# MiniMax-AI/VTP

Measured on AMD Instinct MI355X. Metric: images/sec/node VTP-B f16d64 256x256 train step, higher is better.
Workload: dtype bf16

## Files before the change

### vtp_amd/csrc/attention_resident.hip

```cpp
#include "common.h"
#include <algorithm>
#include <cstdio>
#include <cstdlib>
#include "vtp_hip.h"

namespace vtp {

constexpr float LOG2E_R = 1.4426950408889634f;
constexpr float LN2_R = 0.6931471805599453f;
constexpr int RES_MAXN = 320;
constexpr int RES_SPLIT_COLS = 4;

struct AttnResArgs {
  const bf16 *q, *k, *v, *o, *d_o;
  bf16 *out, *dq, *dk, *dv;
  float* lse;
  float* delta;
  const bf16 *rope_sin, *rope_cos;
  int rope_prefix;
  int B, N, heads, npad;
  long sb, sn, sbo, sno;
  float scale;
  int stagger;
  long long* timing;
// ... 142 lines not shown
  stage_resident(p.k + (long)b * p.sb + h * 64, p.sn, p.N, p.npad, Ks, wave, nwaves, lane);
  stage_resident(p.v + (long)b * p.sb + h * 64, p.sn, p.N, p.npad, Vs, wave, nwaves, lane);
  wait_vmcnt_upto(((p.npad >> 3) - wave + nwaves - 1) / nwaves);
  __builtin_amdgcn_s_barrier();
  asm volatile("" ::: "memory");
  const float sc2 = p.scale * LOG2E_R;
  const int nkb = p.npad >> 5, last = nkb - 1;
  float mx = -INFINITY;
  for (int kb = 0; kb < (active ? nkb : 0); ++kb) {
    f32x16 s;
    zero16r(s);
#pragma unroll
    for (int ks = 0; ks < 4; ++ks) s = __builtin_amdgcn_mfma_f32_32x32x16_bf16(frag_row(Ks, kb * 32, ks, lane), qf[ks], s, 0, 0, 0);
    if (kb == last) {
#pragma unroll
      for (int r = 0; r < 16; ++r)
        if (kb * 32 + (r & 3) + 8 * (r >> 2) + 4 * hi >= p.N) s[r] = -INFINITY;
    }
#pragma unroll
    for (int r = 0; r < 16; ++r) mx = fmaxf(mx, s[r]);
  }
  mx = fmaxf(mx, __shfl_xor(mx, 32, 64));
  const float m2 = mx * sc2;
  wait_all_dma();
  __syncthreads();
  if (!active) return;
  f32x16 oacc[2];
  zero16r(oacc[0]);
  zero16r(oacc[1]);
  float l = 0.f;
  for (int kb = 0; kb < nkb; ++kb) {
    f32x16 s;
    zero16r(s);
#pragma unroll
    for (int ks = 0; ks < 4; ++ks) s = __builtin_amdgcn_mfma_f32_32x32x16_bf16(frag_row(Ks, kb * 32, ks, lane), qf[ks], s, 0, 0, 0);
#pragma unroll
    for (int r = 0; r < 16; ++r) s[r] = fast_exp2(s[r] * sc2 - m2);
    if (kb == last) {
#pragma unroll
      for (int r = 0; r < 16; ++r)
        if (kb * 32 + (r & 3) + 8 * (r >> 2) + 4 * hi >= p.N) s[r] = 0.f;
    }
#pragma unroll
    for (int r = 0; r < 16; ++r) l += s[r];
    const bf16x8 pf0 = pack8r(s, 0), pf1 = pack8r(s, 8);
#pragma unroll
    for (int db = 0; db < 2; ++db) {
      oacc[db] = __builtin_amdgcn_mfma_f32_32x32x16_bf16(frag_tr(Vs, db, kb * 32, 0, lane), pf0, oacc[db], 0, 0, 0);
      oacc[db] = __builtin_amdgcn_mfma_f32_32x32x16_bf16(frag_tr(Vs, db, kb * 32, 1, lane), pf1, oacc[db], 0, 0, 0);
    }
  }
  l += __shfl_xor(l, 32, 64);
  if (qi >= p.N) return;
  const float inv = 1.f / l;
  bf16* orow = p.out + (long)b * p.sbo + (long)qi * p.sno + h * 64;
#pragma unroll
  for (int db = 0; db < 2; ++db)
#pragma unroll
    for (int g = 0; g < 4; ++g) {
      f32x4 v;
#pragma unroll
      for (int e = 0; e < 4; ++e) v[e] = oacc[db][4 * g + e] * inv;
      *(bf16x4*)(orow + db * 32 + 8 * g + 4 * hi) = __builtin_convertvector(v, bf16x4);
    }
  if (hi == 0 && p.lse) p.lse[((long)b * p.heads + h) * p.N + qi] = (m2 + log2f(l)) * LN2_R;
}

__device__ __forceinline__ float both_halves_sum(float x) {
  const auto r = __builtin_amdgcn_permlane32_swap(__float_as_uint(x), __float_as_uint(x), false, false);
  return __uint_as_float(r[0]) + __uint_as_float(r[1]);
}

__device__ __forceinline__ float max3f(float a, float b, float c) {
  float r;
  asm("v_max3_f32 %0, %1, %2, %3" : "=v"(r) : "v"(a), "v"(b), "v"(c));
  return r;
}
__device__ __forceinline__ float max2f(float a, float b) {
  float r;
  asm("v_max_f32 %0, %1, %2" : "=v"(r) : "v"(a), "v"(b));
  return r;
}

constexpr float LAZY_LOG2 = 6.f;

template <int T>
__device__ __forceinline__ void attn_key_loop(const char* Ks, const char* Vs, const bf16x8 (&qf)[T][4], int N, int nkb, int kb0, int step,
                                              float sc2, int lane, f32x16 (&oacc)[T][2], float (&m)[T], float (&l)[T],
                                              int stream_ops = 0) {
  const int hi = lane >> 5, last = nkb - 1;
  const f32x16 zero = {0.f, 0.f, 0.f, 0.f, 0.f, 0.f, 0.f, 0.f, 0.f, 0.f, 0.f, 0.f, 0.f, 0.f, 0.f, 0.f};
  const f32x2 sc2v = {sc2, sc2};
#pragma unroll
  for (int t = 0; t < T; ++t) {
    oacc[t][0] = zero;
    oacc[t][1] = zero;
    m[t] = -INFINITY;
    l[t] = 0.f;
  }
  for (int kb = kb0; kb < nkb; kb += step) {
    if (stream_ops > 0 && (kb == 2 || kb == 5)) {
      wait_vmcnt_upto(__builtin_amdgcn_readfirstlane(kb == 2 ? stream_ops * max(nkb - 5, 0) : 0));
      __builtin_amdgcn_s_barrier();
      asm volatile("" ::: "memory");
    }
    f32x16 s[T];
    {
      bf16x8 kf[4];
#pragma unroll
      for (int ks = 0; ks < 4; ++ks) kf[ks] = frag_row(Ks, kb * 32, ks, lane);
#pragma unroll
      for (int t = 0; t < T; ++t) {
        s[t] = __builtin_amdgcn_mfma_f32_32x32x16_bf16(kf[0], qf[t][0], zero, 0, 0, 0);
#pragma unroll
        for (int ks = 1; ks < 4; ++ks) s[t] = __builtin_amdgcn_mfma_f32_32x32x16_bf16(kf[ks], qf[t][ks], s[t], 0, 0, 0);
      }
    }
    bf16x8 vf[2][2];
#pragma unroll
    for (int db = 0; db < 2; ++db)
#pragma unroll
      for (int ks = 0; ks < 2; ++ks) vf[db][ks] = frag_tr(Vs, db, kb * 32, ks, lane);
    if (kb == last && (N & 31)) {
#pragma unroll
      for (int t = 0; t < T; ++t)
#pragma unroll
        for (int r = 0; r < 16; ++r)
          if (kb * 32 + (r & 3) + 8 * (r >> 2) + 4 * hi >= N) s[t][r] = -INFINITY;
    }
    float mn[T];
    bool moved = false;
#pragma unroll
    for (int t = 0; t < T; ++t) {
      float bm = max3f(s[t][0], s[t][1], s[t][2]);
#pragma unroll
      for (int r = 3; r < 15; r += 2) bm = max3f(bm, s[t][r], s[t][r + 1]);
      bm = max2f(bm, s[t][15]);
      const auto sw = __builtin_amdgcn_permlane32_swap(__float_as_uint(bm), __float_as_uint(bm), false, false);
      bm = max2f(__uint_as_float(sw[0]), __uint_as_float(sw[1]));
      const float cand = bm * sc2;
      mn[t] = cand > m[t] + LAZY_LOG2 ? cand : m[t];
      moved |= mn[t] > m[t];
    }
    if (__any(moved)) {
#pragma unroll
      for (int t = 0; t < T; ++t) {
        const float alpha = fast_exp2(m[t] - mn[t]);
        l[t] *= alpha;
        oacc[t][0] *= alpha;
        oacc[t][1] *= alpha;
        m[t] = mn[t];
      }
    }
    bf16x8 pf[T][2];
#pragma unroll
    for (int t = 0; t < T; ++t) {
      const f32x2 mv = {-m[t], -m[t]};
      f32x2 acc = {0.f, 0.f};
#pragma unroll
      for (int i = 0; i < 8; ++i) {
        f32x2 v = {s[t][2 * i], s[t][2 * i + 1]};
        v = __builtin_elementwise_fma(v, sc2v, mv);
        v[0] = fast_exp2(v[0]);
        v[1] = fast_exp2(v[1]);
        acc += v;
        s[t][2 * i] = v[0];
        s[t][2 * i + 1] = v[1];
      }
      l[t] += acc[0] + acc[1];
      pf[t][0] = pack8r(s[t], 0);
      pf[t][1] = pack8r(s[t], 8);
    }
#pragma unroll
    for (int db = 0; db < 2; ++db)
#pragma unroll
      for (int ks = 0; ks < 2; ++ks) {
#pragma unroll
        for (int t = 0; t < T; ++t) oacc[t][db] = __builtin_amdgcn_mfma_f32_32x32x16_bf16(vf[db][ks], pf[t][ks], oacc[t][db], 0, 0, 0);
      }
  }
}

__device__ __forceinline__ void store_o_row(bf16* orow, const f32x16 (&o)[2], float inv, int hi, bool valid) {
#pragma unroll
  for (int db = 0; db < 2; ++db)
#pragma unroll
    for (int j = 0; j < 2; ++j) {
      uint32_t x[2], y[2];
#pragma unroll
      for (int w = 0; w < 2; ++w) {
        const f32x2 vx = {o[db][8 * j + 2 * w] * inv, o[db][8 * j + 2 * w + 1] * inv};
        const f32x2 vy = {o[db][8 * j + 4 + 2 * w] * inv, o[db][8 * j + 4 + 2 * w + 1] * inv};
        const bf16x2 bx = __builtin_convertvector(vx, bf16x2), by = __builtin_convertvector(vy, bf16x2);
        x[w] = __builtin_bit_cast(uint32_t, bx);
        y[w] = __builtin_bit_cast(uint32_t, by);
      }
      uint32_t out[4];
#pragma unroll
      for (int w = 0; w < 2; ++w) {
        const auto r = __builtin_amdgcn_permlane32_swap(x[w], y[w], false, false);
        out[w] = r[0];
        out[2 + w] = r[1];
      }
      if (valid) {
        typedef __attribute__((ext_vector_type(4))) uint32_t u32x4;
        *(u32x4*)(orow + db * 32 + 16 * j + 8 * hi) = u32x4{out[0], out[1], out[2], out[3]};
      }
    }
}

__device__ __forceinline__ void stage_piece_asm(const bf16* base, long sn, int N, int piece, unsigned img_off, int lane) {
  const int row = piece * 8 + (lane >> 3);
  const int c = (lane & 7) ^ swz_key(row);
  const unsigned voff = (unsigned)(min(row, N - 1) * (int)sn + c * 8) * 2u;
  const unsigned dst = __builtin_amdgcn_readfirstlane(img_off + piece * 1024);
  unsigned keep;
  asm volatile("s_mov_b32 %0, m0\n\ts_mov_b32 m0, %3\n\ts_nop 0\n\tglobal_load_lds_dwordx4 %1, %2\n\ts_mov_b32 m0, %0"
               : "=&s"(keep)
               : "v"(voff), "s"(base), "s"(dst)
               : "memory");
}
__device__ __forceinline__ void stage_block_asm(const bf16* kbase, const bf16* vbase, long sn, int N, int kb, unsigned img, int wave,
                                                int nwaves, int lane) {
  for (int j = wave; j < 4; j += nwaves) {
    stage_piece_asm(kbase, sn, N, kb * 4 + j, 0, lane);
    stage_piece_asm(vbase, sn, N, kb * 4 + j, img, lane);
  }
}

#define ATTN_TSTAMP(i)                                                                            \
  do {                                                                                            \
    if (p.delta && blockIdx.x == 3 && blockIdx.y == 5 && lane == 0)                               \
      ((long long*)p.delta)[wave * 8 + (i)] = __builtin_readcyclecounter();                       \
  } while (0)

__global__ __launch_bounds__(256, 2) void attn_fwd_res2_kernel(const AttnResArgs p) {
  extern __shared__ __attribute__((aligned(16))) char smem[];
  char* Ks = smem;
  char* Vs = smem + p.npad * 128;
  float* part = (float*)(smem + 2 * p.npad * 128);
  const int lane = threadIdx.x & 63, wave = threadIdx.x >> 6, nwaves = blockDim.x >> 6, hi = lane >> 5;
  const int h = blockIdx.x, b = blockIdx.y;
  const bf16* qb = p.q + (long)b * p.sb + h * 64;
  const int ntiles = p.npad >> 5, nkb = ntiles, q0 = wave * 64;
  ATTN_TSTAMP(0);
  const bool split_last = (ntiles & 1) && ntiles > 1;
  const int qL = (ntiles - 1) * 32;
  bf16x8 qf[2][4], qfl[1][4];
#pragma unroll
  for (int t = 0; t < 2; ++t) {
    const bf16* qr = qb + (long)min(q0 + 32 * t + (lane & 31), p.N - 1) * p.sn + hi * 8;
#pragma unroll
    for (int ks = 0; ks < 4; ++ks) qf[t][ks] = *(const bf16x8*)(qr + ks * 16);
  }
  if (split_last) {
    const bf16* qr = qb + (long)min(qL + (lane & 31), p.N - 1) * p.sn + hi * 8;
#pragma unroll
    for (int ks = 0; ks < 4; ++ks) qfl[0][ks] = *(const bf16x8*)(qr + ks * 16);
  }
  const bf16* kbase = p.k + (long)b * p.sb + h * 64;
  const bf16* vbase = p.v + (long)b * p.sb + h * 64;
  const unsigned img = p.npad * 128;
  stage_block_asm(kbase, vbase, p.sn, p.N, 0, img, wave, nwaves, lane);
  if (nkb > 1) stage_block_asm(kbase, vbase, p.sn, p.N, 1, img, wave, nwaves, lane);
  __builtin_amdgcn_s_waitcnt(0x0F70);
  ATTN_TSTAMP(1);
  __builtin_amdgcn_s_barrier();
  asm volatile("" ::: "memory");
  ATTN_TSTAMP(2);
  for (int kb = 2; kb < nkb; ++kb) stage_block_asm(kbase, vbase, p.sn, p.N, kb, img, wave, nwaves, lane);
  const int stream_ops = 2 * ((4 - wave + nwaves - 1) / nwaves);
  const float sc2 = p.scale * LOG2E_R;
  const long srow0 = ((long)b * p.heads + h) * p.N;
  {
    f32x16 oacc[2][2];
    float m[2], l[2];
    const bool two = q0 + 32 < p.npad && !(split_last && q0 + 32 >= qL);
    if (two) attn_key_loop<2>(Ks, Vs, qf, p.N, nkb, 0, 1, sc2, lane, oacc, m, l, stream_ops);
    else {
      f32x16 (&o1)[1][2] = *(f32x16(*)[1][2])&oacc;
      attn_key_loop<1>(Ks, Vs, *(const bf16x8(*)[1][4])&qf, p.N, nkb, 0, 1, sc2, lane, o1, *(float(*)[1])&m, *(float(*)[1])&l,
                       stream_ops);
    }
    ATTN_TSTAMP(3);
#pragma unroll
    for (int t = 0; t < 2; ++t) {
      if (t == 1 && !two) break;
      const int qi = q0 + 32 * t + (lane & 31);
      const float lt = both_halves_sum(l[t]);
      const bool valid = qi < p.N;
      store_o_row(p.out + (long)b * p.sbo + (long)min(qi, p.N - 1) * p.sno + h * 64, oacc[t], 1.f / lt, hi, valid);
      if (valid && hi == 0 && p.lse) p.lse[srow0 + qi] = (m[t] + log2f(lt)) * LN2_R;
    }
  }
  ATTN_TSTAMP(4);
  if (!split_last) return;
  const int cols = p.N - qL;
  {
    f32x16 oacc[1][2];
    float m[1], l[1];
    attn_key_loop<1>(Ks, Vs, qfl, p.N, nkb, wave, nwaves, sc2, lane, oacc, m, l);
    const float lt = both_halves_sum(l[0]);
    if ((lane & 31) < cols) {
      float* dst = part + ((wave * cols + (lane & 31)) * 2 + hi) * 34;
      dst[0] = m[0];
      dst[1] = lt;
#pragma unroll
      for (int r = 0; r < 16; ++r) {
        dst[2 + r] = oacc[0][0][r];
        dst[18 + r] = oacc[0][1][r];
      }
    }
  }
  ATTN_TSTAMP(5);
  __syncthreads();
  ATTN_TSTAMP(6);
  if (wave != 0) return;
  {
    const int c = min(lane & 31, cols - 1);
    float M = -INFINITY;
    for (int w = 0; w < nwaves; ++w) M = fmaxf(M, part[((w * cols + c) * 2 + hi) * 34]);
    f32x16 o[2];
    zero16r(o[0]);
    zero16r(o[1]);
    float L = 0.f;
    for (int w = 0; w < nwaves; ++w) {
      const float* src = part + ((w * cols + c) * 2 + hi) * 34;
      const float sc = fast_exp2(src[0] - M);
      L += src[1] * sc;
#pragma unroll
      for (int r = 0; r < 16; ++r) {
        o[0][r] += src[2 + r] * sc;
        o[1][r] += src[18 + r] * sc;
      }
    }
    const int qi = qL + (lane & 31);
    const bool valid = (lane & 31) < cols;
    store_o_row(p.out + (long)b * p.sbo + (long)min(qi, p.N - 1) * p.sno + h * 64, o, 1.f / L, hi, valid);
    if (valid && hi == 0 && p.lse) p.lse[srow0 + qi] = (M + log2f(L)) * LN2_R;
  }
}

__global__ __launch_bounds__(640) void attn_bwd_dq_res_kernel(const AttnResArgs p) {
  extern __shared__ __attribute__((aligned(16))) char smem[];
  char* Ks = smem;
  char* Vs = smem + p.npad * 128;
  const int lane = threadIdx.x & 63, wave = threadIdx.x >> 6, nwaves = blockDim.x >> 6, hi = lane >> 5;
  const int h = blockIdx.x, b = blockIdx.y;
  BWD_STAMP(0);
  if (__builtin_expect(p.stagger > 0, 0)) {
    const int wg = (blockIdx.z * gridDim.y + blockIdx.y) * gridDim.x + blockIdx.x;
    if (wg < 256 && ((wg >> 3) & 1)) {
      const unsigned long long t0 = wall_clock64();
      while (wall_clock64() - t0 < (unsigned long long)p.stagger) __builtin_amdgcn_s_sleep(16);
    }
  }
  stage_resident(p.k + (long)b * p.sb + h * 64, p.sn, p.N, p.npad, Ks, wave, nwaves, lane);
  stage_resident(p.v + (long)b * p.sb + h * 64, p.sn, p.N, p.npad, Vs, wave, nwaves, lane);
  const int q0 = (blockIdx.z * nwaves + wave) * 32, qi = q0 + (lane & 31), qc = min(qi, p.N - 1);
  bf16x8 qf[4], dof[4];
  {
    const bf16* qr = p.q + (long)b * p.sb + h * 64 + (long)qc * p.sn + hi * 8;
    const bf16* gr = p.d_o + (long)b * p.sbo + h * 64 + (long)qc * p.sno + hi * 8;
#pragma unroll
    for (int ks = 0; ks < 4; ++ks) {
      qf[ks] = *(const bf16x8*)(qr + ks * 16);
      dof[ks] = *(const bf16x8*)(gr + ks * 16);
    }
  }
  const long srow = ((long)b * p.heads + h) * p.N + qc;
  const float lse2 = p.lse[srow] * LOG2E_R;
  float dlt = 0.f;
  {
    const bf16* orow = p.o + (long)b * p.sbo + h * 64 + (long)qc * p.sno + hi * 8;
#pragma unroll
    for (int ks = 0; ks < 4; ++ks) {
      const bf16x8 ov = *(const bf16x8*)(orow + ks * 16);
#pragma unroll
      for (int e = 0; e < 8; ++e) dlt += bf2f(ov[e]) * bf2f(dof[ks][e]);
    }
    dlt += __shfl_xor(dlt, 32, 64);
    if (hi == 0 && qi < p.N) p.delta[srow] = dlt;
  }
  wait_all_dma();
  __syncthreads();
  BWD_STAMP(1);
  if (q0 >= p.npad) return;
  const float sc2 = p.scale * LOG2E_R;
  const f32x2 sc2v = {sc2, sc2}, nlse = {-lse2, -lse2}, scv = {p.scale, p.scale}, ndlt = {-dlt * p.scale, -dlt * p.scale};
  const int nkb = p.npad >> 5, last = nkb - 1;
  f32x16 dq[2];
  zero16r(dq[0]);
  zero16r(dq[1]);
  for (int kb = 0; kb < nkb; ++kb) {
    f32x16 s, dp;
    zero16r(s);
    zero16r(dp);
#pragma unroll
    for (int ks = 0; ks < 4; ++ks) {
      s = __builtin_amdgcn_mfma_f32_32x32x16_bf16(frag_row(Ks, kb * 32, ks, lane), qf[ks], s, 0, 0, 0);
      dp = __builtin_amdgcn_mfma_f32_32x32x16_bf16(frag_row(Vs, kb * 32, ks, lane), dof[ks], dp, 0, 0, 0);
    }
#pragma unroll
    for (int i = 0; i < 8; ++i) {
      f32x2 e = {s[2 * i], s[2 * i + 1]}, g = {dp[2 * i], dp[2 * i + 1]};
      e = __builtin_elementwise_fma(e, sc2v, nlse);
      g = __builtin_elementwise_fma(g, scv, ndlt);
      e[0] = fast_exp2(e[0]);
      e[1] = fast_exp2(e[1]);
      e *= g;
      s[2 * i] = e[0];
      s[2 * i + 1] = e[1];
    }
    if (kb == last && (p.N & 31)) {
#pragma unroll
      for (int r = 0; r < 16; ++r)
        if (kb * 32 + (r & 3) + 8 * (r >> 2) + 4 * hi >= p.N) s[r] = 0.f;
    }
    const bf16x8 d0 = pack8r(s, 0), d1 = pack8r(s, 8);
#pragma unroll
    for (int db = 0; db < 2; ++db) {
      dq[db] = __builtin_amdgcn_mfma_f32_32x32x16_bf16(frag_tr(Ks, db, kb * 32, 0, lane), d0, dq[db], 0, 0, 0);
      dq[db] = __builtin_amdgcn_mfma_f32_32x32x16_bf16(frag_tr(Ks, db, kb * 32, 1, lane), d1, dq[db], 0, 0, 0);
    }
// ... 191 lines not shown
#pragma unroll
  for (int ks = 0; ks < 4; ++ks)
#pragma unroll
    for (int e = 0; e < 8; ++e) dlt += bf2f(of[ks][e]) * bf2f(dof[ks][e]);
  return dlt + __shfl_xor(dlt, 32, 64);
}

#define PB_STAMP(i)                                                                                                   \
  do {                                                                                                                \
    if (__builtin_expect(p.timing != nullptr, 0) && lane == 0) p.timing[((size_t)hid * 16 + wave) * 4 + (i)] = wall_clock64(); \
  } while (0)

__device__ __forceinline__ void dkv_step(const bf16x8 (&kf)[4], const bf16x8 (&vf)[4], f32x16 (&dk)[2], f32x16 (&dv)[2],
                                         const int (&rpart)[4], const int (&tpart)[2][2], int qoff, int img, const float* lse_s,
                                         const float* dlt_s, f32x2 sc2v, f32x2 scv, int q0, int N, bool mask, int hi) {
  f32x16 s, dp;
  zero16r(s);
  zero16r(dp);
#pragma unroll
  for (int ks = 0; ks < 4; ++ks) {
    s = __builtin_amdgcn_mfma_f32_32x32x16_bf16(frag_row_at(lds_addr(rpart[ks], qoff)), kf[ks], s, 0, 0, 0);
    dp = __builtin_amdgcn_mfma_f32_32x32x16_bf16(frag_row_at(lds_addr(rpart[ks], qoff + img)), vf[ks], dp, 0, 0, 0);
  }
  f32x16 pr;
#pragma unroll
  for (int g = 0; g < 4; ++g) {
    const f32x4 l4 = *(const f32x4*)(lse_s + q0 + 8 * g + 4 * hi);
    const f32x4 d4 = *(const f32x4*)(dlt_s + q0 + 8 * g + 4 * hi);
#pragma unroll
    for (int e2 = 0; e2 < 2; ++e2) {
      const int r = 4 * g + 2 * e2;
      f32x2 e = {s[r], s[r + 1]}, gq = {dp[r], dp[r + 1]};
      e = __builtin_elementwise_fma(e, sc2v, f32x2{l4[2 * e2], l4[2 * e2 + 1]});
      gq = __builtin_elementwise_fma(gq, scv, f32x2{d4[2 * e2], d4[2 * e2 + 1]});
      e[0] = fast_exp2(e[0]);
      e[1] = fast_exp2(e[1]);
      if (mask) {
        if (q0 + 8 * g + 4 * hi + 2 * e2 >= N) e[0] = 0.f;
        if (q0 + 8 * g + 4 * hi + 2 * e2 + 1 >= N) e[1] = 0.f;
      }
      pr[r] = e[0];
      pr[r + 1] = e[1];
      e *= gq;
      s[r] = e[0];
      s[r + 1] = e[1];
    }
  }
  const bf16x8 p0 = pack8r(pr, 0), p1 = pack8r(pr, 8), d0 = pack8r(s, 0), d1 = pack8r(s, 8);
#pragma unroll
  for (int db = 0; db < 2; ++db) {
    const int tq0 = lds_addr(tpart[db][0], qoff), tq1 = lds_addr(tpart[db][1], qoff);
    const int tg0 = lds_addr(tpart[db][0], qoff + img), tg1 = lds_addr(tpart[db][1], qoff + img);
    dv[db] = __builtin_amdgcn_mfma_f32_32x32x16_bf16(frag_tr_at(tg0, tg1, 0), p0, dv[db], 0, 0, 0);
    dv[db] = __builtin_amdgcn_mfma_f32_32x32x16_bf16(frag_tr_at(tg0, tg1, 1), p1, dv[db], 0, 0, 0);
    dk[db] = __builtin_amdgcn_mfma_f32_32x32x16_bf16(frag_tr_at(tq0, tq1, 0), d0, dk[db], 0, 0, 0);
    dk[db] = __builtin_amdgcn_mfma_f32_32x32x16_bf16(frag_tr_at(tq0, tq1, 1), d1, dk[db], 0, 0, 0);
  }
}

__device__ __forceinline__ void put_slot(float* slot, const f32x16 (&acc)[2], int hi) {
#pragma unroll
  for (int db = 0; db < 2; ++db)
#pragma unroll
    for (int g = 0; g < 4; ++g) {
      f32x4 v;
#pragma unroll
      for (int e = 0; e < 4; ++e) v[e] = acc[db][4 * g + e];
      *(f32x4*)(slot + 32 * db + 8 * g + 4 * hi) = v;
    }
}
__device__ __forceinline__ void store_acc_rows(bf16* row, const f32x16 (&acc)[2], int hi, const bf16* sin_t, const bf16* cos_t, long t) {
#pragma unroll
  for (int g = 0; g < 4; ++g) {
    f32x4 lo, hv;
#pragma unroll
    for (int e = 0; e < 4; ++e) {
      lo[e] = acc[0][4 * g + e];
      hv[e] = acc[1][4 * g + e];
    }
    store_grad_pair(row, 8 * g + 4 * hi, lo, hv, sin_t, cos_t, t);
  }
}

template <int W>
__global__ __launch_bounds__(64 * W) void attn_bwd_fused_kernel(const AttnResArgs p) {
  extern __shared__ __attribute__((aligned(16))) char smem[];
  const int lane = threadIdx.x & 63, wave = threadIdx.x >> 6, hi = lane >> 5;
  const int img = p.npad * 128, nb = p.npad >> 5, last = nb - 1;
  const bool odd = nb > W;
  const int nx = odd ? p.N - 32 * W : 0;
  const int QO = 0, KO = img, VO = 2 * img, GO = 3 * img;
  float* lse_s = (float*)(smem + 4 * img);
  float* dlt_s = lse_s + p.npad;
  float* xq = dlt_s + p.npad;
  float* xk = xq + (W + 1) * PB_XROWS * 64;
  float* xv = xk + (W + 1) * PB_XROWS * 64;
  const int hid = blockIdx.x, b = hid / p.heads, h = hid - b * p.heads;
  PB_STAMP(0);
  stage_image_asm(p.q + (long)b * p.sb + h * 64, p.sn, p.N, p.npad, QO, wave, W, lane);
  stage_image_asm(p.d_o + (long)b * p.sbo + h * 64, p.sno, p.N, p.npad, GO, wave, W, lane);
  stage_image_asm(p.k + (long)b * p.sb + h * 64, p.sn, p.N, p.npad, KO, wave, W, lane);
  stage_image_asm(p.v + (long)b * p.sb + h * 64, p.sn, p.N, p.npad, VO, wave, W, lane);
  const float sc2 = p.scale * LOG2E_R;
  const f32x2 sc2v = {sc2, sc2}, scv = {p.scale, p.scale};
  int rpart[4], tpart[2][2];
#pragma unroll
  for (int ks = 0; ks < 4; ++ks) rpart[ks] = row_part(lane) ^ (ks << 5);
#pragma unroll
  for (int db = 0; db < 2; ++db)
#pragma unroll
    for (int hf = 0; hf < 2; ++hf) tpart[db][hf] = tr_part(lane, hf) ^ (db << 6);
  const long srow0 = ((long)b * p.heads + h) * p.N;
  const int ri = wave * 32 + (lane & 31);
  const int rx = 32 * W + (lane & 31);
  bf16x8 of[4], of2[4];
  float lse_raw, lse_raw2 = 0.f;
  {
    const int qc = min(ri, p.N - 1);
    const bf16* orow = p.o + (long)b * p.sbo + h * 64 + (long)qc * p.sno + hi * 8;
#pragma unroll
    for (int ks = 0; ks < 4; ++ks) of[ks] = *(const bf16x8*)(orow + ks * 16);
    lse_raw = p.lse[srow0 + qc];
    if (odd) {
      const int qc2 = min(rx, p.N - 1);
      const bf16* orow2 = p.o + (long)b * p.sbo + h * 64 + (long)qc2 * p.sno + hi * 8;
#pragma unroll
      for (int ks = 0; ks < 4; ++ks) of2[ks] = *(const bf16x8*)(orow2 + ks * 16);
      lse_raw2 = p.lse[srow0 + qc2];
    }
  }
  wait_all_dma();
  __syncthreads();
  PB_STAMP(1);
  {
    bf16x8 qf[4], dof[4];
    const int own = __builtin_amdgcn_readfirstlane(wave * 4096);
#pragma unroll
    for (int ks = 0; ks < 4; ++ks) {
      qf[ks] = frag_row_at(lds_addr(rpart[ks], QO + own));
      dof[ks] = frag_row_at(lds_addr(rpart[ks], GO + own));
    }
    const float dlt = row_delta(of, dof);
    if (hi == 0) {
      lse_s[ri] = -lse_raw * LOG2E_R;
      dlt_s[ri] = -dlt * p.scale;
      if (ri < p.N) p.delta[srow0 + ri] = dlt;
    }
    {
      const float lse2 = lse_raw * LOG2E_R;
      const f32x2 nlse = {-lse2, -lse2}, ndlt = {-dlt * p.scale, -dlt * p.scale};
      f32x16 dq[2];
      zero16r(dq[0]);
      zero16r(dq[1]);
      for (int kb = 0; kb < nb; ++kb)
        dq_step(qf, dof, dq, rpart, tpart, __builtin_amdgcn_readfirstlane(KO + kb * 4096), img, sc2v, nlse, scv, ndlt, kb * 32, p.N,
                kb == last && (p.N & 31), hi);
      if (ri < p.N) {
        const bool rot = p.rope_sin && ri >= p.rope_prefix;
        store_acc_rows(p.dq + (long)b * p.sb + (long)ri * p.sn + h * 64, dq, hi, rot ? p.rope_sin : nullptr, p.rope_cos,
                       (long)(ri - p.rope_prefix) * 64);
      }
    }
    if (odd) {
      const int ox = __builtin_amdgcn_readfirstlane(W * 4096);
#pragma unroll
      for (int ks = 0; ks < 4; ++ks) {
        qf[ks] = frag_row_at(lds_addr(rpart[ks], QO + ox));
        dof[ks] = frag_row_at(lds_addr(rpart[ks], GO + ox));
      }
      const float dlt2 = row_delta(of2, dof);
      if (wave == 0 && hi == 0) {
        lse_s[rx] = -lse_raw2 * LOG2E_R;
        dlt_s[rx] = -dlt2 * p.scale;
        if (rx < p.N) p.delta[srow0 + rx] = dlt2;
      }
      const float lse2 = lse_raw2 * LOG2E_R;
      const f32x2 nlse = {-lse2, -lse2}, ndlt = {-dlt2 * p.scale, -dlt2 * p.scale};
      for (int kb = wave; kb < nb; kb += W) {
        f32x16 dqx[2];
        zero16r(dqx[0]);
        zero16r(dqx[1]);
        dq_step(qf, dof, dqx, rpart, tpart, __builtin_amdgcn_readfirstlane(KO + kb * 4096), img, sc2v, nlse, scv, ndlt, kb * 32, p.N,
                kb == last && (p.N & 31), hi);
        if ((lane & 31) < nx) put_slot(xq + (kb * PB_XROWS + (lane & 31)) * 64, dqx, hi);
      }
    }
  }
  __syncthreads();
  PB_STAMP(2);
  if (odd && (int)threadIdx.x < nx * 8) {
    const int row = threadIdx.x >> 3, d0 = 4 * (threadIdx.x & 7), qrow = 32 * W + row;
    f32x4 lo = {0.f, 0.f, 0.f, 0.f}, hv = {0.f, 0.f, 0.f, 0.f};
    for (int kb = 0; kb < nb; ++kb) {
      lo += *(const f32x4*)(xq + (kb * PB_XROWS + row) * 64 + d0);
      hv += *(const f32x4*)(xq + (kb * PB_XROWS + row) * 64 + 32 + d0);
    }
    const bool rot = p.rope_sin && qrow >= p.rope_prefix;
    store_grad_pair(p.dq + (long)b * p.sb + (long)qrow * p.sn + h * 64, d0, lo, hv, rot ? p.rope_sin : nullptr, p.rope_cos,
                    (long)(qrow - p.rope_prefix) * 64);
  }
  {
    bf16x8 kf[4], vf[4];
    const int own = __builtin_amdgcn_readfirstlane(wave * 4096);
#pragma unroll
    for (int ks = 0; ks < 4; ++ks) {
      kf[ks] = frag_row_at(lds_addr(rpart[ks], KO + own));
      vf[ks] = frag_row_at(lds_addr(rpart[ks], VO + own));
    }
    {
      f32x16 dk[2], dv[2];
      zero16r(dk[0]);
      zero16r(dk[1]);
      zero16r(dv[0]);
      zero16r(dv[1]);
      for (int qb = 0; qb < nb; ++qb)
        dkv_step(kf, vf, dk, dv, rpart, tpart, __builtin_amdgcn_readfirstlane(QO + qb * 4096), GO - QO, lse_s, dlt_s, sc2v, scv, qb * 32,
                 p.N, qb == last && (p.N & 31), hi);
      if (ri < p.N) {
        const bool rot = p.rope_sin && ri >= p.rope_prefix;
        store_acc_rows(p.dk + (long)b * p.sb + (long)ri * p.sn + h * 64, dk, hi, rot ? p.rope_sin : nullptr, p.rope_cos,
                       (long)(ri - p.rope_prefix) * 64);
        store_acc_rows(p.dv + (long)b * p.sb + (long)ri * p.sn + h * 64, dv, hi, nullptr, nullptr, 0);
      }
    }
    if (odd) {
      const int ox = __builtin_amdgcn_readfirstlane(W * 4096);
#pragma unroll
      for (int ks = 0; ks < 4; ++ks) {
        kf[ks] = frag_row_at(lds_addr(rpart[ks], KO + ox));
        vf[ks] = frag_row_at(lds_addr(rpart[ks], VO + ox));
      }
      for (int qb = wave; qb < nb; qb += W) {
        f32x16 dkx[2], dvx[2];
        zero16r(dkx[0]);
        zero16r(dkx[1]);
        zero16r(dvx[0]);
        zero16r(dvx[1]);
        dkv_step(kf, vf, dkx, dvx, rpart, tpart, __builtin_amdgcn_readfirstlane(QO + qb * 4096), GO - QO, lse_s, dlt_s, sc2v, scv,
                 qb * 32, p.N, qb == last && (p.N & 31), hi);
        if ((lane & 31) < nx) {
          put_slot(xk + (qb * PB_XROWS + (lane & 31)) * 64, dkx, hi);
          put_slot(xv + (qb * PB_XROWS + (lane & 31)) * 64, dvx, hi);
        }
      }
    }
  }
  if (odd) {
    __syncthreads();
    if ((int)threadIdx.x < nx * 8) {
      const int row = threadIdx.x >> 3, d0 = 4 * (threadIdx.x & 7), krow_i = 32 * W + row;
      f32x4 lo = {0.f, 0.f, 0.f, 0.f}, hv = lo, c0 = lo, c1 = lo;
      for (int qb = 0; qb < nb; ++qb) {
        lo += *(const f32x4*)(xk + (qb * PB_XROWS + row) * 64 + d0);
        hv += *(const f32x4*)(xk + (qb * PB_XROWS + row) * 64 + 32 + d0);
        c0 += *(const f32x4*)(xv + (qb * PB_XROWS + row) * 64 + d0);
        c1 += *(const f32x4*)(xv + (qb * PB_XROWS + row) * 64 + 32 + d0);
      }
      const bool rot = p.rope_sin && krow_i >= p.rope_prefix;
      store_grad_pair(p.dk + (long)b * p.sb + (long)krow_i * p.sn + h * 64, d0, lo, hv, rot ? p.rope_sin : nullptr, p.rope_cos,
                      (long)(krow_i - p.rope_prefix) * 64);
      store_grad_pair(p.dv + (long)b * p.sb + (long)krow_i * p.sn + h * 64, d0, c0, c1, nullptr, nullptr, 0);
    }
  }
  PB_STAMP(3);
}

static int res_waves_per_block(int nw, int groups) {
  return (groups <= 512 && nw >= 4) ? (nw + 1) / 2 : nw;
}

template <typename K>
static void set_lds(K kern, int bytes) {
  hipFuncSetAttribute((const void*)kern, hipFuncAttributeMaxDynamicSharedMemorySize, bytes);
}

static long long* g_attn_timing = nullptr;
static int g_attn_wpb = 0;
static int g_attn_lds_pad = 0;
static int g_attn_stagger = 0;

int attn_resident_fwd(const void* q, const void* k, const void* v, void* o, float* lse, int B, int N, int heads, long sb,
                      long sn, long sbo, long sno, float scale, hipStream_t s) {
  AttnResArgs a = {};
  a.q = (const bf16*)q; a.k = (const bf16*)k; a.v = (const bf16*)v; a.out = (bf16*)o; a.lse = lse;
  a.B = B; a.N = N; a.heads = heads; a.npad = (N + 31) / 32 * 32; a.sb = sb; a.sn = sn; a.sbo = sbo; a.sno = sno; a.scale = scale;
  static bool attr = false;
  if (!attr) {
    set_lds(attn_fwd_res_kernel, 2 * RES_MAXN * 128);
    set_lds(attn_fwd_res2_kernel, 2 * RES_MAXN * 128 + 5 * RES_SPLIT_COLS * 2 * 34 * 4);
    attr = true;
  }
  {
    const int ntiles = a.npad / 32, cols = N - 32 * (ntiles - 1);
    const bool odd = (ntiles & 1) && ntiles > 1;
    if (!odd || cols <= RES_SPLIT_COLS) {
      const int waves = std::max(1, ntiles / 2);
      const int lds = 2 * a.npad * 128 + (odd ? waves * cols * 2 * 34 * 4 : 0);
      static long long* tbuf = nullptr;
      static const bool timing = getenv("VTP_ATTN_TIMING") != nullptr;
      if (timing && !tbuf && hipMalloc((void**)&tbuf, 64 * 8) != hipSuccess) tbuf = nullptr;
      if (timing) a.delta = (float*)tbuf;
      hipLaunchKernelGGL(attn_fwd_res2_kernel, dim3(heads, B), dim3(64 * waves), lds, s, a);
      if (timing && tbuf) {
        int occ = -1;
        (void)hipOccupancyMaxActiveBlocksPerMultiprocessor(&occ, attn_fwd_res2_kernel, 64 * waves, lds);
        fprintf(stderr, "[attn timing] workgroups per CU by the runtime's count: %d (lds %d B, %d waves)\n", occ, lds, waves);
        long long hbuf[64];
        (void)hipStreamSynchronize(s);
        (void)hipMemcpy(hbuf, tbuf, sizeof hbuf, hipMemcpyDeviceToHost);
        for (int w = 0; w < waves; ++w) {
          fprintf(stderr, "[attn timing] wave %d:", w);
          for (int i = 1; i < 7; ++i) fprintf(stderr, " t%d=%lld", i, hbuf[w * 8 + i] - hbuf[0]);
          fprintf(stderr, "\n");
        }
      }
      return check_launch("attn_fwd_resident2");
    }
  }
  const int nw = a.npad / 32, wpb = res_waves_per_block(nw, heads * B);
  hipLaunchKernelGGL(attn_fwd_res_kernel, dim3(heads, B, (nw + wpb - 1) / wpb), dim3(64 * wpb), 2 * a.npad * 128, s, a);
  return check_launch("attn_fwd_resident");
}

int attn_resident_bwd(const void* q, const void* k, const void* v, const void* o, const void* d_o, const float* lse,
                      float* delta, void* dq, void* dk, void* dv, const void* rope_sin, const void* rope_cos, int rope_prefix,
                      int B, int N, int heads, long sb, long sn, long sbo, long sno, float scale, hipStream_t s) {
  AttnResArgs a = {};
  a.q = (const bf16*)q; a.k = (const bf16*)k; a.v = (const bf16*)v; a.o = (const bf16*)o; a.d_o = (const bf16*)d_o;
  a.lse = (float*)lse; a.delta = delta; a.dq = (bf16*)dq; a.dk = (bf16*)dk; a.dv = (bf16*)dv;
  a.rope_sin = (const bf16*)rope_sin; a.rope_cos = (const bf16*)rope_cos; a.rope_prefix = rope_prefix;
  a.B = B; a.N = N; a.heads = heads; a.npad = (N + 31) / 32 * 32; a.sb = sb; a.sn = sn; a.sbo = sbo; a.sno = sno; a.scale = scale;
  a.timing = g_attn_timing;
  a.stagger = g_attn_stagger;
  static bool attr = false;
  if (!attr) {
    set_lds(attn_bwd_dq_res_kernel, 2 * RES_MAXN * 128 + 32768);
    set_lds(attn_bwd_dkv_res_kernel, 2 * RES_MAXN * 128 + 8 * RES_MAXN + 32768);
    attr = true;
  }
  const int nw = a.npad / 32;
  auto fits = [&](int W) { return nw == W || (nw == W + 1 && N - 32 * W <= PB_XROWS); };
  const bool off32 = (long)N * sn * 2 < (1L << 31) && (long)N * sno * 2 < (1L << 31);
  if (g_attn_wpb == 0 && off32 && (fits(PB_WAVES) || fits(2))) {
    auto lds_of = [](int npad, int W) { return 4 * npad * 128 + 8 * npad + 3 * (W + 1) * PB_XROWS * 256; };
    static bool attr_p = false;
    if (!attr_p) {
      set_lds(attn_bwd_fused_kernel<PB_WAVES>, lds_of(32 * (PB_WAVES + 1), PB_WAVES));
      set_lds(attn_bwd_fused_kernel<2>, lds_of(32 * 3, 2));
      attr_p = true;
    }
    if (fits(PB_WAVES))
      hipLaunchKernelGGL(attn_bwd_fused_kernel<PB_WAVES>, dim3(B * heads), dim3(64 * PB_WAVES), lds_of(a.npad, PB_WAVES), s, a);
    else
      hipLaunchKernelGGL(attn_bwd_fused_kernel<2>, dim3(B * heads), dim3(128), lds_of(a.npad, 2), s, a);
    return check_launch("attn_bwd_fused");
  }
  const int wpb = g_attn_wpb > 0 ? std::min(g_attn_wpb, nw) : res_waves_per_block(nw, heads * B);
  const dim3 grid(heads, B, (nw + wpb - 1) / wpb), block(64 * wpb);
  if (a.timing) {
    int o1 = -1, o2 = -1;
    (void)hipOccupancyMaxActiveBlocksPerMultiprocessor(&o1, attn_bwd_dq_res_kernel, block.x, 2 * a.npad * 128);
    (void)hipOccupancyMaxActiveBlocksPerMultiprocessor(&o2, attn_bwd_dkv_res_kernel, block.x, 2 * a.npad * 128 + 8 * a.npad);
    fprintf(stderr, "[attn timing] workgroups per CU by the runtime's count: dQ %d, dK/dV %d (%d waves, lds %d / %d B)\n", o1, o2,
            (int)block.x / 64, 2 * a.npad * 128, 2 * a.npad * 128 + 8 * a.npad);
  }
  hipLaunchKernelGGL(attn_bwd_dq_res_kernel, grid, block, 2 * a.npad * 128 + g_attn_lds_pad, s, a);
  if (a.timing) a.timing += (size_t)grid.x * grid.y * grid.z * 64;
  hipLaunchKernelGGL(attn_bwd_dkv_res_kernel, grid, block, 2 * a.npad * 128 + 8 * a.npad + g_attn_lds_pad, s, a);
  return check_launch("attn_bwd_resident");
}

}

extern "C" int vtp_attn_debug(void* timing, int lds_pad, int waves_per_wg, int stagger_ticks) {
  vtp::g_attn_stagger = stagger_ticks;
  vtp::g_attn_wpb = waves_per_wg;
  vtp::g_attn_timing = (long long*)timing;
  vtp::g_attn_lds_pad = lds_pad;
  return 0;
}
```

Measured before the change: 738.4.

## Handle single extra key row with scalar path instead of padded tile

When N is one more than a multiple of 32 (e.g. 256 patches plus a CLS token), forward and fused backward attention kernels now process only the full 32-row tiles with MFMA. The leftover single row is folded in with scalar dot/axpy code in LDS, replacing a mostly empty padded 32-row tile. In the backward kernel the leftover row's dQ/dK/dV contributions are gathered through small column MFMAs and a final cross-wave reduction. This avoids nearly a whole tile of wasted MFMA and staging work, at the cost of more code complexity and some serialized scalar work.

Measured after the change: 741.3 (median of 6 runs). No clear change (+0.4%).

```diff
diff --git a/vtp_amd/csrc/attention_resident.hip b/vtp_amd/csrc/attention_resident.hip
--- a/vtp_amd/csrc/attention_resident.hip
+++ b/vtp_amd/csrc/attention_resident.hip
@@ -248,6 +248,33 @@
   return r;
 }
 
+__device__ __forceinline__ float sb_dot(const bf16x8 (&f)[4], int row, int hi) {
+  float acc = 0.f;
+#pragma unroll
+  for (int ks = 0; ks < 4; ++ks) {
+    const bf16x8 x = *(const __attribute__((address_space(3))) bf16x8*)(size_t)(row + (2 * ks + hi) * 16);
+#pragma unroll
+    for (int j = 0; j < 4; ++j)
+      acc = __builtin_amdgcn_fdot2_f32_bf16(bf16x2{f[ks][2 * j], f[ks][2 * j + 1]}, bf16x2{x[2 * j], x[2 * j + 1]}, acc, false);
+  }
+  return both_halves_sum(acc);
+}
+__device__ __forceinline__ void sb_axpy(f32x16 (&acc)[2], float a, int row, int hi) {
+#pragma unroll
+  for (int db = 0; db < 2; ++db)
+#pragma unroll
+    for (int g = 0; g < 4; ++g) {
+      const bf16x4 x = *(const __attribute__((address_space(3))) bf16x4*)(size_t)(row + (32 * db + 8 * g + 4 * hi) * 2);
+#pragma unroll
+      for (int e = 0; e < 4; ++e) acc[db][4 * g + e] = __builtin_fmaf(a, bf2f(x[e]), acc[db][4 * g + e]);
+    }
+}
+__device__ __forceinline__ bf16x8 col_operand(const float* c, int ks, int hi) {
+  const f32x4 a = *(const f32x4*)(c + 16 * ks + 4 * hi), b = *(const f32x4*)(c + 16 * ks + 4 * hi + 8);
+  const bf16x4 ab = __builtin_convertvector(a, bf16x4), bb = __builtin_convertvector(b, bf16x4);
+  return __builtin_shufflevector(ab, bb, 0, 1, 2, 3, 4, 5, 6, 7);
+}
+
 constexpr float LAZY_LOG2 = 6.f;
 
 template <int T>
@@ -344,6 +371,36 @@
 #pragma unroll
         for (int t = 0; t < T; ++t) oacc[t][db] = __builtin_amdgcn_mfma_f32_32x32x16_bf16(vf[db][ks], pf[t][ks], oacc[t][db], 0, 0, 0);
       }
+  }
+}
+
+template <int T>
+__device__ __forceinline__ void sb_key_fold(const bf16x8 (&qf)[T][4], int kx, int vx, float sc2, int hi, f32x16 (&oacc)[T][2],
+                                            float (&m)[T], float (&l)[T]) {
+  float s[T], mn[T];
+  bool moved = false;
+#pragma unroll
+  for (int t = 0; t < T; ++t) {
+    s[t] = sb_dot(qf[t], kx, hi);
+    const float cand = s[t] * sc2;
+    mn[t] = cand > m[t] + LAZY_LOG2 ? cand : m[t];
+    moved |= mn[t] > m[t];
+  }
+  if (__any(moved)) {
+#pragma unroll
+    for (int t = 0; t < T; ++t) {
+      const float alpha = fast_exp2(m[t] - mn[t]);
+      l[t] *= alpha;
+      oacc[t][0] *= alpha;
+      oacc[t][1] *= alpha;
+      m[t] = mn[t];
+    }
+  }
+#pragma unroll
+  for (int t = 0; t < T; ++t) {
+    const float pr = fast_exp2(__builtin_fmaf(s[t], sc2, -m[t]));
+    l[t] += hi ? 0.f : pr;
+    sb_axpy(oacc[t], bf2f(f2bf(pr)), vx, hi);
   }
 }
 
@@ -400,17 +457,20 @@
       ((long long*)p.delta)[wave * 8 + (i)] = __builtin_readcyclecounter();                       \
   } while (0)
 
-__global__ __launch_bounds__(256, 2) void attn_fwd_res2_kernel(const AttnResArgs p) {
+template <bool SB>
+__device__ __forceinline__ void attn_fwd_res2_body(const AttnResArgs p) {
   extern __shared__ __attribute__((aligned(16))) char smem[];
+  const int rows = SB ? p.N + 7 : p.npad;
   char* Ks = smem;
-  char* Vs = smem + p.npad * 128;
-  float* part = (float*)(smem + 2 * p.npad * 128);
+  char* Vs = smem + rows * 128;
+  float* part = (float*)(smem + 2 * rows * 128);
   const int lane = threadIdx.x & 63, wave = threadIdx.x >> 6, nwaves = blockDim.x >> 6, hi = lane >> 5;
   const int h = blockIdx.x, b = blockIdx.y;
   const bf16* qb = p.q + (long)b * p.sb + h * 64;
-  const int ntiles = p.npad >> 5, nkb = ntiles, q0 = wave * 64;
+  const int ntiles = p.npad >> 5, nkb = SB ? ntiles - 1 : ntiles, q0 = wave * 64;
+  const int nmask = SB ? p.N - 1 : p.N;
   ATTN_TSTAMP(0);
-  const bool split_last = (ntiles & 1) && ntiles > 1;
+  const bool split_last = SB || ((ntiles & 1) && ntiles > 1);
   const int qL = (ntiles - 1) * 32;
   bf16x8 qf[2][4], qfl[1][4];
 #pragma unroll
@@ -426,9 +486,13 @@
   }
   const bf16* kbase = p.k + (long)b * p.sb + h * 64;
   const bf16* vbase = p.v + (long)b * p.sb + h * 64;
-  const unsigned img = p.npad * 128;
+  const unsigned img = rows * 128;
   stage_block_asm(kbase, vbase, p.sn, p.N, 0, img, wave, nwaves, lane);
   if (nkb > 1) stage_block_asm(kbase, vbase, p.sn, p.N, 1, img, wave, nwaves, lane);
+  if (SB && wave == 0) {
+    stage_piece_asm(kbase, p.sn, p.N, 4 * nkb, 0, lane);
+    stage_piece_asm(vbase, p.sn, p.N, 4 * nkb, img, lane);
+  }
   __builtin_amdgcn_s_waitcnt(0x0F70);
   ATTN_TSTAMP(1);
   __builtin_amdgcn_s_barrier();
@@ -442,11 +506,16 @@
     f32x16 oacc[2][2];
     float m[2], l[2];
     const bool two = q0 + 32 < p.npad && !(split_last && q0 + 32 >= qL);
-    if (two) attn_key_loop<2>(Ks, Vs, qf, p.N, nkb, 0, 1, sc2, lane, oacc, m, l, stream_ops);
-    else {
+    if (two) {
+      attn_key_loop<2>(Ks, Vs, qf, nmask, nkb, 0, 1, sc2, lane, oacc, m, l, stream_ops);
+      if constexpr (SB) sb_key_fold<2>(qf, (p.N - 1) * 128, img + (p.N - 1) * 128, sc2, hi, oacc, m, l);
+    } else {
       f32x16 (&o1)[1][2] = *(f32x16(*)[1][2])&oacc;
-      attn_key_loop<1>(Ks, Vs, *(const bf16x8(*)[1][4])&qf, p.N, nkb, 0, 1, sc2, lane, o1, *(float(*)[1])&m, *(float(*)[1])&l,
+      attn_key_loop<1>(Ks, Vs, *(const bf16x8(*)[1][4])&qf, nmask, nkb, 0, 1, sc2, lane, o1, *(float(*)[1])&m, *(float(*)[1])&l,
                        stream_ops);
+      if constexpr (SB)
+        sb_key_fold<1>(*(const bf16x8(*)[1][4])&qf, (p.N - 1) * 128, img + (p.N - 1) * 128, sc2, hi, o1, *(float(*)[1])&m,
+                       *(float(*)[1])&l);
     }
     ATTN_TSTAMP(3);
 #pragma unroll
@@ -465,7 +534,8 @@
   {
     f32x16 oacc[1][2];
     float m[1], l[1];
-    attn_key_loop<1>(Ks, Vs, qfl, p.N, nkb, wave, nwaves, sc2, lane, oacc, m, l);
+    attn_key_loop<1>(Ks, Vs, qfl, nmask, nkb, wave, nwaves, sc2, lane, oacc, m, l);
+    if (SB && wave == 0) sb_key_fold<1>(qfl, (p.N - 1) * 128, img + (p.N - 1) * 128, sc2, hi, oacc, m, l);
     const float lt = both_halves_sum(l[0]);
     if ((lane & 31) < cols) {
       float* dst = part + ((wave * cols + (lane & 31)) * 2 + hi) * 34;
@@ -506,6 +576,8 @@
     if (valid && hi == 0 && p.lse) p.lse[srow0 + qi] = (M + log2f(L)) * LN2_R;
   }
 }
+__global__ __launch_bounds__(256, 2) void attn_fwd_res2_kernel(const AttnResArgs p) { attn_fwd_res2_body<false>(p); }
+__global__ __launch_bounds__(256, 2) void attn_fwd_res2_sb_kernel(const AttnResArgs p) { attn_fwd_res2_body<true>(p); }
 
 __global__ __launch_bounds__(640) void attn_bwd_dq_res_kernel(const AttnResArgs p) {
   extern __shared__ __attribute__((aligned(16))) char smem[];
@@ -863,25 +935,31 @@
   }
 }
 
-template <int W>
-__global__ __launch_bounds__(64 * W) void attn_bwd_fused_kernel(const AttnResArgs p) {
+template <int W, bool SB>
+__device__ __forceinline__ void attn_bwd_fused_body(const AttnResArgs p) {
   extern __shared__ __attribute__((aligned(16))) char smem[];
   const int lane = threadIdx.x & 63, wave = threadIdx.x >> 6, hi = lane >> 5;
-  const int img = p.npad * 128, nb = p.npad >> 5, last = nb - 1;
-  const bool odd = nb > W;
+  const int rows = SB ? 32 * W + 8 : p.npad;
+  const int img = rows * 128, nb = SB ? W : p.npad >> 5, last = nb - 1;
+  const bool odd = !SB && nb > W;
   const int nx = odd ? p.N - 32 * W : 0;
   const int QO = 0, KO = img, VO = 2 * img, GO = 3 * img;
   float* lse_s = (float*)(smem + 4 * img);
-  float* dlt_s = lse_s + p.npad;
-  float* xq = dlt_s + p.npad;
+  float* dlt_s = lse_s + rows;
+  float* xq = dlt_s + rows;
   float* xk = xq + (W + 1) * PB_XROWS * 64;
   float* xv = xk + (W + 1) * PB_XROWS * 64;
+  float* pcol = xv + (W + 1) * PB_XROWS * 64;
+  float* dcol = pcol + 32 * W;
+  float* dxcol = dcol + 32 * W;
+  float* sbx = dxcol + 32 * W;
+  const int xoff = 32 * W * 128;
   const int hid = blockIdx.x, b = hid / p.heads, h = hid - b * p.heads;
   PB_STAMP(0);
-  stage_image_asm(p.q + (long)b * p.sb + h * 64, p.sn, p.N, p.npad, QO, wave, W, lane);
-  stage_image_asm(p.d_o + (long)b * p.sbo + h * 64, p.sno, p.N, p.npad, GO, wave, W, lane);
-  stage_image_asm(p.k + (long)b * p.sb + h * 64, p.sn, p.N, p.npad, KO, wave, W, lane);
-  stage_image_asm(p.v + (long)b * p.sb + h * 64, p.sn, p.N, p.npad, VO, wave, W, lane);
+  stage_image_asm(p.q + (long)b * p.sb + h * 64, p.sn, p.N, rows, QO, wave, W, lane);
+  stage_image_asm(p.d_o + (long)b * p.sbo + h * 64, p.sno, p.N, rows, GO, wave, W, lane);
+  stage_image_asm(p.k + (long)b * p.sb + h * 64, p.sn, p.N, rows, KO, wave, W, lane);
+  stage_image_asm(p.v + (long)b * p.sb + h * 64, p.sn, p.N, rows, VO, wave, W, lane);
   const float sc2 = p.scale * LOG2E_R;
   const f32x2 sc2v = {sc2, sc2}, scv = {p.scale, p.scale};
   int rpart[4], tpart[2][2];
@@ -902,7 +980,7 @@
 #pragma unroll
     for (int ks = 0; ks < 4; ++ks) of[ks] = *(const bf16x8*)(orow + ks * 16);
     lse_raw = p.lse[srow0 + qc];
-    if (odd) {
+    if (odd || SB) {
       const int qc2 = min(rx, p.N - 1);
       const bf16* orow2 = p.o + (long)b * p.sbo + h * 64 + (long)qc2 * p.sno + hi * 8;
 #pragma unroll
@@ -933,13 +1011,44 @@
       f32x16 dq[2];
       zero16r(dq[0]);
       zero16r(dq[1]);
+      if constexpr (SB) {
+        const float s = sb_dot(qf, KO + xoff, hi), dp = sb_dot(dof, VO + xoff, hi);
+        const float pr = fast_exp2(__builtin_fmaf(s, sc2, -lse2)), ds = pr * __builtin_fmaf(dp, p.scale, -dlt * p.scale);
+        sb_axpy(dq, bf2f(f2bf(ds)), KO + xoff, hi);
+        if (hi == 0) {
+          pcol[ri] = pr;
+          dcol[ri] = ds;
+        }
+      }
       for (int kb = 0; kb < nb; ++kb)
         dq_step(qf, dof, dq, rpart, tpart, __builtin_amdgcn_readfirstlane(KO + kb * 4096), img, sc2v, nlse, scv, ndlt, kb * 32, p.N,
-                kb == last && (p.N & 31), hi);
+                !SB && kb == last && (p.N & 31), hi);
       if (ri < p.N) {
         const bool rot = p.rope_sin && ri >= p.rope_prefix;
         store_acc_rows(p.dq + (long)b * p.sb + (long)ri * p.sn + h * 64, dq, hi, rot ? p.rope_sin : nullptr, p.rope_cos,
                        (long)(ri - p.rope_prefix) * 64);
+      }
+    }
+    if constexpr (SB) {
+      f32x16 ck[2], cv[2];
+      zero16r(ck[0]);
+      zero16r(ck[1]);
+      zero16r(cv[0]);
+      zero16r(cv[1]);
+#pragma unroll
+      for (int ks = 0; ks < 2; ++ks) {
+        const bf16x8 bp = col_operand(pcol + wave * 32, ks, hi), bd = col_operand(dcol + wave * 32, ks, hi);
+#pragma unroll
+        for (int db = 0; db < 2; ++db) {
+          cv[db] = __builtin_amdgcn_mfma_f32_32x32x16_bf16(
+              frag_tr_at(lds_addr(tpart[db][0], GO + own), lds_addr(tpart[db][1], GO + own), ks), bp, cv[db], 0, 0, 0);
+          ck[db] = __builtin_amdgcn_mfma_f32_32x32x16_bf16(
+              frag_tr_at(lds_addr(tpart[db][0], QO + own), lds_addr(tpart[db][1], QO + own), ks), bd, ck[db], 0, 0, 0);
+        }
+      }
+      if ((lane & 31) == 0) {
+        put_slot(xk + wave * 64, ck, hi);
+        put_slot(xv + wave * 64, cv, hi);
       }
     }
     if (odd) {
@@ -994,15 +1103,52 @@
       zero16r(dk[1]);
       zero16r(dv[0]);
       zero16r(dv[1]);
+      if constexpr (SB) {
+        const float dltx = sb_dot(of2, GO + xoff, hi), lse2x = lse_raw2 * LOG2E_R;
+        const float s = sb_dot(kf, QO + xoff, hi), dp = sb_dot(vf, GO + xoff, hi);
+        const float pr = fast_exp2(__builtin_fmaf(s, sc2, -lse2x)), ds = pr * __builtin_fmaf(dp, p.scale, -dltx * p.scale);
+        sb_axpy(dv, bf2f(f2bf(pr)), GO + xoff, hi);
+        sb_axpy(dk, bf2f(f2bf(ds)), QO + xoff, hi);
+        if (hi == 0) dxcol[ri] = ds;
+        if (wave == 0) {
+          bf16x8 xf[4];
+#pragma unroll
+          for (int ks = 0; ks < 4; ++ks) xf[ks] = *(const __attribute__((address_space(3))) bf16x8*)(size_t)(QO + xoff + (2 * ks + hi) * 16);
+          const float sxx = sb_dot(xf, KO + xoff, hi);
+#pragma unroll
+          for (int ks = 0; ks < 4; ++ks) xf[ks] = *(const __attribute__((address_space(3))) bf16x8*)(size_t)(GO + xoff + (2 * ks + hi) * 16);
+          const float dpxx = sb_dot(xf, VO + xoff, hi);
+          if (lane == 0) {
+            const float pxx = fast_exp2(__builtin_fmaf(sxx, sc2, -lse2x));
+            sbx[0] = pxx;
+            sbx[1] = pxx * __builtin_fmaf(dpxx, p.scale, -dltx * p.scale);
+            p.delta[srow0 + p.N - 1] = dltx;
+          }
+        }
+      }
       for (int qb = 0; qb < nb; ++qb)
         dkv_step(kf, vf, dk, dv, rpart, tpart, __builtin_amdgcn_readfirstlane(QO + qb * 4096), GO - QO, lse_s, dlt_s, sc2v, scv, qb * 32,
-                 p.N, qb == last && (p.N & 31), hi);
+                 p.N, !SB && qb == last && (p.N & 31), hi);
       if (ri < p.N) {
         const bool rot = p.rope_sin && ri >= p.rope_prefix;
         store_acc_rows(p.dk + (long)b * p.sb + (long)ri * p.sn + h * 64, dk, hi, rot ? p.rope_sin : nullptr, p.rope_cos,
                        (long)(ri - p.rope_prefix) * 64);
         store_acc_rows(p.dv + (long)b * p.sb + (long)ri * p.sn + h * 64, dv, hi, nullptr, nullptr, 0);
       }
+    }
+    if constexpr (SB) {
+      f32x16 cq[2];
+      zero16r(cq[0]);
+      zero16r(cq[1]);
+#pragma unroll
+      for (int ks = 0; ks < 2; ++ks) {
+        const bf16x8 bd = col_operand(dxcol + wave * 32, ks, hi);
+#pragma unroll
+        for (int db = 0; db < 2; ++db)
+          cq[db] = __builtin_amdgcn_mfma_f32_32x32x16_bf16(
+              frag_tr_at(lds_addr(tpart[db][0], KO + own), lds_addr(tpart[db][1], KO + own), ks), bd, cq[db], 0, 0, 0);
+      }
+      if ((lane & 31) == 0) put_slot(xq + wave * 64, cq, hi);
     }
     if (odd) {
       const int ox = __builtin_amdgcn_readfirstlane(W * 4096);
@@ -1043,8 +1189,36 @@
       store_grad_pair(p.dv + (long)b * p.sb + (long)krow_i * p.sn + h * 64, d0, c0, c1, nullptr, nullptr, 0);
     }
   }
+  if constexpr (SB) {
+    __syncthreads();
+    if (threadIdx.x < 24) {
+      const int which = threadIdx.x >> 3, d0 = 4 * (threadIdx.x & 7), x = p.N - 1;
+      const float* slot = which == 0 ? xq : which == 1 ? xk : xv;
+      f32x4 lo = {0.f, 0.f, 0.f, 0.f}, hv = lo;
+      for (int w = 0; w < W; ++w) {
+        lo += *(const f32x4*)(slot + w * 64 + d0);
+        hv += *(const f32x4*)(slot + w * 64 + 32 + d0);
+      }
+      const float a = bf2f(f2bf(sbx[which == 2 ? 0 : 1]));
+      const int row = (which == 0 ? KO : which == 1 ? QO : GO) + xoff;
+      const bf16x4 r0 = *(const __attribute__((address_space(3))) bf16x4*)(size_t)(row + d0 * 2);
+      const bf16x4 r1 = *(const __attribute__((address_space(3))) bf16x4*)(size_t)(row + (32 + d0) * 2);
+#pragma unroll
+      for (int e = 0; e < 4; ++e) {
+        lo[e] = __builtin_fmaf(a, bf2f(r0[e]), lo[e]);
+        hv[e] = __builtin_fmaf(a, bf2f(r1[e]), hv[e]);
+      }
+      bf16* dst = (which == 0 ? p.dq : which == 1 ? p.dk : p.dv) + (long)b * p.sb + (long)x * p.sn + h * 64;
+      const bool rot = which < 2 && p.rope_sin && x >= p.rope_prefix;
+      store_grad_pair(dst, d0, lo, hv, rot ? p.rope_sin : nullptr, p.rope_cos, (long)(x - p.rope_prefix) * 64);
+    }
+  }
   PB_STAMP(3);
 }
+template <int W>
+__global__ __launch_bounds__(64 * W) void attn_bwd_fused_kernel(const AttnResArgs p) { attn_bwd_fused_body<W, false>(p); }
+template <int W>
+__global__ __launch_bounds__(64 * W) void attn_bwd_fused_sb_kernel(const AttnResArgs p) { attn_bwd_fused_body<W, true>(p); }
 
 static int res_waves_per_block(int nw, int groups) {
   return (groups <= 512 && nw >= 4) ? (nw + 1) / 2 : nw;
@@ -1069,22 +1243,26 @@
   if (!attr) {
     set_lds(attn_fwd_res_kernel, 2 * RES_MAXN * 128);
     set_lds(attn_fwd_res2_kernel, 2 * RES_MAXN * 128 + 5 * RES_SPLIT_COLS * 2 * 34 * 4);
+    set_lds(attn_fwd_res2_sb_kernel, 2 * (256 + 8) * 128 + 4 * 2 * 34 * 4);
     attr = true;
   }
   {
     const int ntiles = a.npad / 32, cols = N - 32 * (ntiles - 1);
     const bool odd = (ntiles & 1) && ntiles > 1;
-    if (!odd || cols <= RES_SPLIT_COLS) {
-      const int waves = std::max(1, ntiles / 2);
-      const int lds = 2 * a.npad * 128 + (odd ? waves * cols * 2 * 34 * 4 : 0);
+    const bool sb = (N & 31) == 1 && N > 1 && N <= 257;
+    if (sb || ((!odd || cols <= RES_SPLIT_COLS) && ntiles <= 9)) {
+      const int waves = sb ? (N / 32 + 1) / 2 : std::max(1, ntiles / 2);
+      const int lds = sb ? 2 * (N + 7) * 128 + waves * 2 * 34 * 4 : 2 * a.npad * 128 + (odd ? waves * cols * 2 * 34 * 4 : 0);
       static long long* tbuf = nullptr;
       static const bool timing = getenv("VTP_ATTN_TIMING") != nullptr;
       if (timing && !tbuf && hipMalloc((void**)&tbuf, 64 * 8) != hipSuccess) tbuf = nullptr;
       if (timing) a.delta = (float*)tbuf;
-      hipLaunchKernelGGL(attn_fwd_res2_kernel, dim3(heads, B), dim3(64 * waves), lds, s, a);
+      if (sb) hipLaunchKernelGGL(attn_fwd_res2_sb_kernel, dim3(heads, B), dim3(64 * waves), lds, s, a);
+      else hipLaunchKernelGGL(attn_fwd_res2_kernel, dim3(heads, B), dim3(64 * waves), lds, s, a);
       if (timing && tbuf) {
         int occ = -1;
-        (void)hipOccupancyMaxActiveBlocksPerMultiprocessor(&occ, attn_fwd_res2_kernel, 64 * waves, lds);
+        (void)hipOccupancyMaxActiveBlocksPerMultiprocessor(&occ, sb ? attn_fwd_res2_sb_kernel : attn_fwd_res2_kernel,
+                                                           64 * waves, lds);
         fprintf(stderr, "[attn timing] workgroups per CU by the runtime's count: %d (lds %d B, %d waves)\n", occ, lds, waves);
         long long hbuf[64];
         (void)hipStreamSynchronize(s);
@@ -1124,16 +1302,23 @@
   const bool off32 = (long)N * sn * 2 < (1L << 31) && (long)N * sno * 2 < (1L << 31);
   if (g_attn_wpb == 0 && off32 && (fits(PB_WAVES) || fits(2))) {
     auto lds_of = [](int npad, int W) { return 4 * npad * 128 + 8 * npad + 3 * (W + 1) * PB_XROWS * 256; };
+    auto lds_sb = [&](int W) { return lds_of(32 * W + 8, W) + 3 * 32 * W * 4 + 2 * 4; };
     static bool attr_p = false;
     if (!attr_p) {
       set_lds(attn_bwd_fused_kernel<PB_WAVES>, lds_of(32 * (PB_WAVES + 1), PB_WAVES));
       set_lds(attn_bwd_fused_kernel<2>, lds_of(32 * 3, 2));
+      set_lds(attn_bwd_fused_sb_kernel<PB_WAVES>, lds_sb(PB_WAVES));
+      set_lds(attn_bwd_fused_sb_kernel<2>, lds_sb(2));
       attr_p = true;
     }
-    if (fits(PB_WAVES))
-      hipLaunchKernelGGL(attn_bwd_fused_kernel<PB_WAVES>, dim3(B * heads), dim3(64 * PB_WAVES), lds_of(a.npad, PB_WAVES), s, a);
+    if (N == 32 * PB_WAVES + 1)
+      hipLaunchKernelGGL((attn_bwd_fused_sb_kernel<PB_WAVES>), dim3(B * heads), dim3(64 * PB_WAVES), lds_sb(PB_WAVES), s, a);
+    else if (fits(PB_WAVES))
+      hipLaunchKernelGGL((attn_bwd_fused_kernel<PB_WAVES>), dim3(B * heads), dim3(64 * PB_WAVES), lds_of(a.npad, PB_WAVES), s, a);
+    else if (N == 32 * 2 + 1)
+      hipLaunchKernelGGL((attn_bwd_fused_sb_kernel<2>), dim3(B * heads), dim3(128), lds_sb(2), s, a);
     else
-      hipLaunchKernelGGL(attn_bwd_fused_kernel<2>, dim3(B * heads), dim3(128), lds_of(a.npad, 2), s, a);
+      hipLaunchKernelGGL((attn_bwd_fused_kernel<2>), dim3(B * heads), dim3(128), lds_of(a.npad, 2), s, a);
     return check_launch("attn_bwd_fused");
   }
   const int wpb = g_attn_wpb > 0 ? std::min(g_attn_wpb, nw) : res_waves_per_block(nw, heads * B);
```
